# UoB-HPC/pbf-sph

Measured on AMD Instinct MI355X. Metric: particle-steps/sec (1 M particles, 4 iters) + achieved HBM GB/s, 1/2/4/8 MI355X, higher is better.
Workload: dtype f32; 1 GPU; dam-break, 1024000 particles (nominal 1048576), box 4600^3, h=0.1, K=4, dt=0.01245, scale=500; timed = simulation frames [200, 2687) after 195 settle + 5 warm-up frames; particles=1024000, solver_iter=4, settle_frames=195, math=precise (IEEE div/sqrt, no contraction), parallelism=1 GPU, device-resident

## Files before the change

include/pbf_hip.h:

```cpp
#ifndef PBF_HIP_H
#define PBF_HIP_H

#include <stddef.h>
#include <stdint.h>

#ifdef __cplusplus
extern "C" {
#endif

#define PBF_ABI_VERSION 1

typedef struct pbf_ctx pbf_ctx;

typedef enum pbf_status {
  PBF_OK = 0,
  PBF_ERR_INVALID = -1,
  PBF_ERR_HIP = -2,
  PBF_ERR_NO_DEVICE = -3,
  PBF_ERR_STATE = -4,
  PBF_ERR_COMM = -5,
} pbf_status;

enum { PBF_TYPE_FLUID = 0, PBF_TYPE_OBSTACLE = 1 };

// ... 50 lines not shown

int pbf_stage_predict(pbf_ctx *ctx, const pbf_params *params);
int pbf_stage_sort(pbf_ctx *ctx, const pbf_params *params);
int pbf_stage_diffuse(pbf_ctx *ctx, const pbf_params *params);
int pbf_stage_lambda(pbf_ctx *ctx, const pbf_params *params);
int pbf_stage_delta(pbf_ctx *ctx, const pbf_params *params);
int pbf_stage_finalise(pbf_ctx *ctx, const pbf_params *params);

enum pbf_buffer {
  PBF_BUF_KEYS = 0,
  PBF_BUF_TABLE = 1,
  PBF_BUF_PSTAR = 2,
  PBF_BUF_NBR_COUNT = 3,
  PBF_BUF_OMEGA = 4,
  PBF_BUF_SURFACE = 5,
  PBF_BUF_COUNT_ = 6,
};
int pbf_read_buffer(pbf_ctx *ctx, int which, void *host, size_t bytes);
size_t pbf_table_size(const pbf_ctx *ctx);
int pbf_grid_extent(const pbf_ctx *ctx, uint64_t extent[3], double min_extent[3]);

int pbf_selftest_math(pbf_ctx *ctx, uint64_t mismatches[4]);

int pbf_stage_times(pbf_ctx *ctx, const char **names, double *mean_ms, uint64_t *calls, int cap);
int pbf_reset_stage_times(pbf_ctx *ctx);

typedef struct pbf_mc_params {
  double resolution, isolevel, particle_size, particle_influence;
} pbf_mc_params;
int pbf_surface(pbf_ctx *ctx, const pbf_params *params, const pbf_mc_params *mc, uint64_t *n_triangles);
int pbf_download_mesh(pbf_ctx *ctx, void *vs, void *ns, void *cs);
// ... 55 lines not shown
```

pbf-sph_amd/capi.py:

```python
import ctypes as C
import os
import subprocess

import numpy as np

PKG_DIR = os.path.dirname(os.path.abspath(__file__))
LIB_PATH = os.environ.get("PBF_HIP_LIB") or os.path.join(PKG_DIR, "libpbf_hip.so")

ABI_VERSION = 1
FLAG_STAGE_TIMING = 1 << 0
FLAG_FAST_MATH = 1 << 1
FLAG_NO_LDS = 1 << 2

BUF_KEYS, BUF_TABLE, BUF_PSTAR = 0, 1, 2
BUF_NBR_COUNT = 3
BUF_OMEGA = 4
BUF_SURFACE = 5


class PbfError(RuntimeError):
    pass


class Desc(C.Structure):
    _fields_ = [
        ("abi_version", C.c_uint32),
        ("fp64", C.c_int32),
        ("device", C.c_int32),
        ("flags", C.c_uint32),
        ("h", C.c_double),
        ("stream", C.c_void_p),
    ]
# ... 278 lines not shown
    def nbr_counts(self):
        k = np.empty(self.n, np.uint32)
        self._chk(self.L.pbf_read_buffer(self.ctx, BUF_NBR_COUNT, _vp(k), k.nbytes), "read neighbour counts")
        return np.where(k == 0xFFFFFFFF, k, k & 0xFF).astype(np.uint32)

    def keys(self):
        k = np.empty(self.n, np.uint32)
        self._chk(self.L.pbf_read_buffer(self.ctx, BUF_KEYS, _vp(k), k.nbytes), "read keys")
        return k

    def table(self):
        t = np.empty(self.L.pbf_table_size(self.ctx), np.uint32)
        self._chk(self.L.pbf_read_buffer(self.ctx, BUF_TABLE, _vp(t), t.nbytes), "read table")
        return t

    def pstar(self):
        a = np.empty((self.n, 4), self.dtype)
        self._chk(self.L.pbf_read_buffer(self.ctx, BUF_PSTAR, _vp(a), a.nbytes), "read pstar")
        return a

    def omega(self):
        a = np.empty((self.n, 4), self.dtype)
        self._chk(self.L.pbf_read_buffer(self.ctx, BUF_OMEGA, _vp(a), a.nbytes), "read omega")
        return a[:, :3].copy()

    def surface(self, p, mc=None):
        mc = mc or McParams()
        nt = C.c_uint64()
        self._chk(self.L.pbf_surface(self.ctx, C.byref(p), C.byref(mc), C.byref(nt)), "pbf_surface")
        n = nt.value
# ... 25 lines not shown
```

pbf-sph_amd/csrc/pbf_hip.hip:

```cpp
#include "pbf_hip.h"

#include <hip/hip_runtime.h>

#include <cmath>
#include <cstdio>
#include <cstdlib>
#include <cstring>
#include <algorithm>
#include <map>
#include <string>
#include <vector>

#include "pbf_kernels.hpp"
#include "pbf_slab.hpp"
#include "pbf_tiles.hpp"
#include "pbf_mc.hpp"
#include "pbf_comm.hpp"

using namespace pbf;

namespace {

thread_local std::string g_create_error;

struct DevBuf {
  void *p = nullptr;
  size_t cap = 0;
  template <typename T> T *as() const { return static_cast<T *>(p); }
};

constexpr uint32_t kTickets = 254;
constexpr int kBrickZ = 4;

enum Stage { ST_PREDICT = 0, ST_SORT, ST_DIFFUSE, ST_LAMBDA, ST_DELTA, ST_FINALISE, ST_BUILD, ST_COUNT };
const char *kStageNames[ST_COUNT] = {"advect+zindex",      "sortz+gridtable", "sph-diffuse",
                                     "sph-lambda",         "sph-delta",       "sph-finalise",
                                     "sph-lambda/list-build"};

struct EventPair {
  hipEvent_t a, b;
  int stage;
};

}

struct StepState {
// ... 274 lines not shown

int ensure_table(pbf_ctx *ctx, uint32_t tableN) {
  const size_t entries = size_t(tableN) + 2;
  if (ctx->tableCap >= entries) return PBF_OK;
  ctx->count.cap = 0;
  if (ctx->count.p) {
    HIPCHK(ctx, hipStreamSynchronize(ctx->stream));
    HIPCHK(ctx, hipFree(ctx->count.p));
    ctx->count.p = nullptr;
  }
  if (int rc = ensure(ctx, ctx->count, (entries + SCAN_TILE) * 4, true)) return rc;
  if (int rc = ensure(ctx, ctx->table, (entries + SCAN_TILE) * 4)) return rc;
  const size_t nb = (entries + SCAN_TILE - 1) / SCAN_TILE + 1;
  if (int rc = ensure(ctx, ctx->blockSums, nb * 4)) return rc;
  if (int rc = ensure(ctx, ctx->bricks, (entries / Brick<kBrickZ>::HOME + 2) * 4)) return rc;
  if (int rc = ensure(ctx, ctx->brickCtl, (kTickets + 2) * 4)) return rc;
  ctx->tableCap = ctx->count.cap / 4 - SCAN_TILE;
  return PBF_OK;
}

hipEvent_t get_event(pbf_ctx *ctx) {
  if (!ctx->freeEvents.empty()) {
    hipEvent_t e = ctx->freeEvents.back();
    ctx->freeEvents.pop_back();
    return e;
  }
  hipEvent_t e = nullptr;
  (void)hipEventCreate(&e);
  return e;
}
int resolve_events(pbf_ctx *ctx) {
// ... 92 lines not shown
  ctx->bricksValid = true;
}

void launch_scans(pbf_ctx *ctx, const ScanJobs &jobs, int njobs, uint32_t *zero = nullptr, uint32_t nZero = 0) {
  const uint32_t blocks = jobs.nb[0] + (njobs > 1 ? jobs.nb[1] : 0u);
  hipLaunchKernelGGL(k_scan_block_sums, dim3(blocks), dim3(BLOCK), 0, ctx->stream, jobs);
  hipLaunchKernelGGL(k_scan_sums, dim3(uint32_t(njobs)), dim3(BLOCK), 0, ctx->stream, jobs, zero, nZero);
  hipLaunchKernelGGL(k_scan_apply, dim3(blocks), dim3(BLOCK), 0, ctx->stream, jobs);
}
ScanJobs scan_job(const uint32_t *count, uint32_t len, uint32_t *sums, uint32_t *table) {
  ScanJobs j{};
  j.count[0] = count, j.sums[0] = sums, j.table[0] = table, j.len[0] = len, j.nb[0] = (len + SCAN_TILE - 1) / SCAN_TILE;
  return j;
}

template <typename N> int stage_sort(pbf_ctx *ctx, const pbf_params *p) {
  if (!ctx->counted) return fail(ctx, PBF_ERR_STATE, "pbf_stage_sort needs pbf_stage_predict first");
  StepConsts<N> c;
  if (int rc = make_consts<N>(ctx, p, c)) return rc;
  if (c.tableN != ctx->countedTableN) return fail(ctx, PBF_ERR_STATE, "bounds changed between predict and sort");
  StageTimer t(ctx, ST_SORT);
  const uint32_t len = c.tableN + 2;
  const uint32_t nb = (len + SCAN_TILE - 1) / SCAN_TILE;
  uint32_t *count = ctx->count.as<uint32_t>(), *table = ctx->table.as<uint32_t>(),
           *sums = ctx->blockSums.as<uint32_t>();
  ScanJobs jobs = scan_job(count, len, sums, table);
  int njobs = 1;
  (void)nb;
  const int s = ctx->cur, d = 1 - s;
  RowArrays<N> row{};
  ctx->rowsValid = false, ctx->pstarInRows = false, ctx->rowsCurrent = false, ctx->rowColValid = false;
  if (row_mode(ctx)) {
    uint32_t pshift = 1;
    while (pshift < 10 && (uint64_t(1) << (3 * pshift)) < uint64_t(c.tableN)) ++pshift;
    const size_t ncells = size_t(1) << (3 * pshift), llen = ncells + 1;
    const uint32_t lnb = uint32_t((llen + SCAN_TILE - 1) / SCAN_TILE);
    const size_t v = sizeof(vec4<N>);
    if (int rc = ensure(ctx, ctx->linCount, (ncells + 2 + SCAN_TILE) * 4)) return rc;
    if (int rc = ensure(ctx, ctx->linTable, (ncells + 2 + SCAN_TILE) * 4)) return rc;
    if (int rc = ensure(ctx, ctx->linSums, (size_t(lnb) + 2) * 4)) return rc;
    for (int k = 0; k < 2; ++k)
      if (int rc = ensure(ctx, ctx->rowPstar[k], ctx->cap * v)) return rc;
    if (int rc = ensure(ctx, ctx->rowMass, ctx->cap * sizeof(N))) return rc;
    if (int rc = ensure(ctx, ctx->rowQpos, (ctx->cap + QPOS_PAD) * 8)) return rc;
    if (int rc = ensure(ctx, ctx->rowXYZ, ctx->cap * 4)) return rc;
    if (int rc = ensure(ctx, ctx->rowType, ctx->cap)) return rc;
    if (int rc = ensure(ctx, ctx->rowSlotOf, ctx->cap * 4)) return rc;
    const bool rowDiffuse = ctx->cellDiffuse && ctx->rowDiffuse > 0;
    const uint32_t segShift = std::min<uint32_t>(pshift, 6u);
    const size_t nSegTotal = ncells >> segShift;
    if (rowDiffuse) {
      if (int rc = ensure(ctx, ctx->rowCol, ctx->cap * v)) return rc;
      if (int rc = ensure(ctx, ctx->rowMortonOf, ctx->cap * 4)) return rc;
      if (int rc = ensure(ctx, ctx->rowSegs, (std::min(nSegTotal, ctx->cap) + 1) * 4)) return rc;
    }
    hipLaunchKernelGGL(k_lin_count, grid_for(ncells + 1), dim3(BLOCK), 0, ctx->stream, c.tableN, pshift, count,
                       ctx->linCount.as<uint32_t>());
    jobs.count[1] = ctx->linCount.as<const uint32_t>(), jobs.sums[1] = ctx->linSums.as<uint32_t>(), jobs.table[1] = ctx->linTable.as<uint32_t>();
    jobs.len[1] = uint32_t(llen), jobs.nb[1] = lnb;
    njobs = 2;
    launch_scans(ctx, jobs, njobs, ctx->brickCtl.as<uint32_t>(), kTickets + 2);
    if (rowDiffuse)
      hipLaunchKernelGGL(k_row_segments, grid_for(nSegTotal), dim3(BLOCK), 0, ctx->stream, pshift, segShift,
                         ctx->linTable.as<const uint32_t>(), ctx->rowSegs.as<uint32_t>(), ctx->linCount.as<uint32_t>() + ncells + 2);
    ctx->rcur = 0;
    row = RowArrays<N>{ctx->rowPstar[0].as<vec4<N>>(), ctx->rowMass.as<N>(), ctx->rowQpos.as<uint2>(), ctx->rowXYZ.as<uint32_t>(),
                       ctx->rowType.as<uint8_t>(), ctx->rowSlotOf.as<uint32_t>(),
                       rowDiffuse ? ctx->rowCol.as<vec4<N>>() : nullptr, rowDiffuse ? ctx->rowMortonOf.as<uint32_t>() : nullptr,
                       ctx->linTable.as<const uint32_t>(), ctx->linCount.as<uint32_t>() + ncells + 1, pshift};
    ctx->rowShift = pshift, ctx->rowSegShift = segShift;
    ctx->rowColValid = rowDiffuse;
    ctx->rowsValid = true, ctx->rowsCurrent = true;
  }
  if (njobs == 1) launch_scans(ctx, jobs, 1, ctx->brickCtl.as<uint32_t>(), kTickets + 2);
  uint32_t *nBig = ctx->brickCtl.as<uint32_t>() + kTickets + 1;
  if (int rc = ensure(ctx, ctx->bigCells, (ctx->cap / BIG_CELL + 2) * 4)) return rc;
  hipLaunchKernelGGL(k_scatter_slots, grid_for(ctx->n), dim3(BLOCK), 0, ctx->stream, c.n, c.tableN,
                     ctx->key[s].as<const uint32_t>(), table, count, ctx->permTmp.as<uint32_t>(),
                     ctx->bigCells.as<uint32_t>(), nBig);
  hipLaunchKernelGGL(k_sort_big_cells, dim3(64), dim3(BLOCK), 0, ctx->stream, table, c.tableN,
                     ctx->bigCells.as<const uint32_t>(), nBig, ctx->permTmp.as<uint32_t>(),
                     ctx->key[s].as<const uint32_t>());
  const size_t nLive = ctx->slabStepMode ? ctx->sortLive : ctx->n;
  hipLaunchKernelGGL((k_rank_move<N>), grid_for(nLive), dim3(BLOCK), 0, ctx->stream, c, uint32_t(nLive), c.tableN,
                     ctx->permTmp.as<const uint32_t>(), table, arrays<N>(ctx, s, s), arrays<N>(ctx, d, d),
                     ctx->slabActive ? ctx->slotOf.as<uint32_t>() : nullptr, ctx->qpos.as<uint2>(), row);
  ctx->n = nLive;
  ctx->gatherSeq = 0;
  ctx->bricksValid = false;
  if (!ctx->rowColValid) brick_list(ctx, c.tableN, true);
  LAUNCH_CHECK(ctx);
  ctx->cur = d;
  ctx->pcur = d;
  ctx->sorted = true;
  ctx->nbrValid = false;
  ctx->qposValid = true;
  if (ctx->rowsValid) ctx->pstarInRows = true, ctx->qposValid = false;
  ctx->counted = false;
  return PBF_OK;
}
// ... 158 lines not shown
  return PBF_OK;
}

template <typename N> int stage_diffuse(pbf_ctx *ctx, const pbf_params *p, bool overlap = false) {
  StepConsts<N> c;
  if (int rc = make_consts<N>(ctx, p, c)) return rc;
  const int s = ctx->cur, d = 1 - s;
  typename DiffuseOp<N>::Args args{ctx->col4[s].as<const vec4<N>>(), ctx->col4[d].as<vec4<N>>(),
                                   ctx->type[s].as<const uint8_t>()};
  const bool timed = (ctx->desc.flags & PBF_FLAG_STAGE_TIMING) != 0 && ((ctx->timingMask >> ST_DIFFUSE) & 1u) != 0;
  overlap = overlap && ctx->overlapDiffuse && ctx->cellDiffuse && !(ctx->desc.flags & PBF_FLAG_NO_LDS) && !timed &&
            (ctx->overlapDiffuseForced || ctx->n >= (size_t(1) << 19));
  ctx->omegaValid = false, ctx->surfaceValid = false;
  StageTimer t(ctx, ST_DIFFUSE);
  if (ctx->cellDiffuse && ctx->rowColValid && ctx->rowsValid && ctx->rowDiffuse) {
    const uint32_t ncells = 1u << (3u * ctx->rowShift);
    const uint32_t cap = ctx->diffuseCap ? ctx->diffuseCap : 640u;
    const size_t lds = size_t(cap + 8) * sizeof(vec4<N>) + size_t(DIFFUSE_ROW_THREADS) * (4 * sizeof(N) + 4) + cap + 8;
    static size_t attrSet = 0;
    if (lds > attrSet) {
      (void)hipFuncSetAttribute(reinterpret_cast<const void *>(k_diffuse_rows<N>), hipFuncAttributeMaxDynamicSharedMemorySize, int(lds));
      attrSet = lds;
    }
    const uint32_t perCU = uint32_t(std::max<size_t>(1, std::min<size_t>(16, (160 * 1024) / (lds + 256))));
    const uint32_t blocks = std::max(8u, (uint32_t(ctx->numCUs) * perCU) & ~7u);
    hipLaunchKernelGGL((k_diffuse_rows<N>), dim3(blocks), dim3(DIFFUSE_ROW_THREADS), lds, ctx->stream, c,
                       row_walk<N>(ctx), ctx->rowCol.as<const vec4<N>>(), ctx->rowType.as<const uint8_t>(),
                       ctx->rowMortonOf.as<const uint32_t>(), ctx->rowSegs.as<const uint32_t>(),
                       ctx->linCount.as<const uint32_t>() + ncells + 2, ctx->rowSegShift, args.colOut, cap, uint32_t(ctx->n));
    LAUNCH_CHECK(ctx);
    ctx->rowColValid = false;
  } else if (ctx->cellDiffuse && !(ctx->desc.flags & PBF_FLAG_NO_LDS)) {
    brick_list(ctx, c.tableN);
    vec4<N> *cellSum = ctx->pstar[other_pstar(ctx)].as<vec4<N>>();
    uint32_t *cellCnt = ctx->nbrCount.as<uint32_t>();
    hipStream_t st = ctx->stream;
    uint32_t cap = 3072u;
    if (overlap) cap = 2048u;
    const size_t lds = Brick<4>::HDR + size_t(cap) * sizeof(vec4<N>);
    uint32_t perCU = uint32_t((160 * 1024) / (lds + 1024));
    if (overlap) {
      if (int rc = ensure(ctx, ctx->diffSum, ctx->cap * sizeof(vec4<N>))) return rc;
      if (int rc = ensure(ctx, ctx->diffCnt, ctx->cap * 4)) return rc;
      if (!ctx->sideStream) {
// ... 243 lines not shown
    std::swap(ctx->pstar[ctx->pcur], ctx->pstar[s]);
    ctx->pcur = s;
  }
  ctx->nbrValid = false;
  if (extras_on(ctx, p)) return extras<N>(ctx, p, c);
  return PBF_OK;
}

template <typename N> int step_impl(pbf_ctx *ctx, const pbf_params *p) {
  if (ctx->n == 0) return PBF_OK;
  if (ctx->prePredicted) {
    ctx->prePredicted = false;
  } else if (int rc = stage_predict<N>(ctx, p)) {
    return rc;
  }
  if (int rc = stage_sort<N>(ctx, p)) return rc;
  const bool fuse = ctx->fuseDiffuse && p->iteration > 0 && ctx->gatherKind == 1 && ctx->reuseLists &&
                    !(ctx->desc.flags & PBF_FLAG_NO_LDS);
  if (!fuse) {
    if (int rc = stage_diffuse<N>(ctx, p, p->iteration > 0)) return rc;
  }
  ctx->fuseDiffuseNow = fuse;
  for (uint64_t it = 0; it < p->iteration; ++it) {
    if (int rc = stage_lambda<N>(ctx, p)) return rc;
    if (int rc = stage_delta<N>(ctx, p)) return rc;
  }
  if (int rc = stage_finalise<N>(ctx, p)) return rc;
  return join_diffuse(ctx);
}

int check(pbf_ctx *ctx, const pbf_params *p, bool needSorted) {
  if (!ctx) return PBF_ERR_INVALID;
  if (!p) return fail(ctx, PBF_ERR_INVALID, "params == NULL");
// ... 542 lines not shown
      src = ctx->table.p, avail = size_t(ctx->tableN) * 4;
      break;
    case PBF_BUF_PSTAR:
      if (int rc = ctx->fp64 ? materialise_pstar<double>(ctx) : materialise_pstar<float>(ctx)) return rc;
      src = ctx->pstar[ctx->pcur].p, avail = ctx->n * v;
      break;
    case PBF_BUF_NBR_COUNT: src = ctx->nbrCount.p, avail = (ctx->ghostsPending ? ctx->nOwned : ctx->n) * 4; break;
    case PBF_BUF_OMEGA:
      if (!ctx->omegaValid) return fail(ctx, PBF_ERR_STATE, "no vorticity pass since the arrays last changed (pbf_params.vorticity)");
      src = ctx->pstar[2].p, avail = ctx->n * v;
      break;
    case PBF_BUF_SURFACE:
      if (!ctx->surfaceValid) return fail(ctx, PBF_ERR_STATE, "no surface-tension pass since the arrays last changed (pbf_set_surface_tension)");
      src = ctx->surfB.p, avail = std::min(ctx->n * v, ctx->surfB.cap);
      break;
    default: return fail(ctx, PBF_ERR_INVALID, "unknown buffer");
  }
  if (bytes > avail) return fail(ctx, PBF_ERR_INVALID, "read beyond buffer");
  if (!src) return fail(ctx, PBF_ERR_STATE, "buffer not allocated yet");
  HIPCHK(ctx, hipMemcpyAsync(host, src, bytes, hipMemcpyDeviceToHost, ctx->stream));
  HIPCHK(ctx, hipStreamSynchronize(ctx->stream));
  return PBF_OK;
}

int pbf_selftest_math(pbf_ctx *ctx, uint64_t mismatches[4]) {
  if (!ctx || !mismatches) return PBF_ERR_INVALID;
  HIPCHK(ctx, hipSetDevice(ctx->device));
  if (int rc = ensure(ctx, ctx->selTotals, 64)) return rc;
  HIPCHK(ctx, hipMemsetAsync(ctx->selTotals.p, 0, 32, ctx->stream));
  if (ctx->fp64) {
// ... 808 lines not shown
```

pbf-sph_amd/csrc/pbf_kernels.hpp:

```cpp
#pragma once

#include <type_traits>

#include "pbf_common.hpp"

namespace pbf {

constexpr int BLOCK = 256;

template <typename N> __device__ inline int64_t cell_coord(N v) {
  return static_cast<int64_t>(v);
}

template <typename F> __device__ inline void wave_bucket_atomic(uint32_t bucket, F &&leader_op, uint32_t &before, uint32_t &rank) {
  const uint32_t lane = threadIdx.x & 63u;
  const uint64_t below = (1ull << lane) - 1ull;
  bool pending = true;
  uint32_t cnt = 0, leader = lane;
  rank = 0;
  while (__any(pending)) {
    if (pending) {
      const uint32_t b = __builtin_amdgcn_readfirstlane(bucket);
      if (bucket == b) {
        const uint64_t same = __ballot(1);
// ... 107 lines not shown
  const uint32_t incl = wave_incl_scan(v, lane);
  __syncthreads();
  if (lane == 63) waveSum[wave] = incl;
  __syncthreads();
  uint32_t off = 0, tot = 0;
#pragma unroll
  for (int w = 0; w < THREADS / 64; ++w) {
    const uint32_t s = waveSum[w];
    if (w < wave) off += s;
    tot += s;
  }
  *total = tot;
  return off + incl - v;
}

struct ScanJobs {
  const uint32_t *count[2];
  uint32_t *sums[2];
  uint32_t *table[2];
  uint32_t len[2], nb[2];
};
__global__ __launch_bounds__(BLOCK) void k_scan_block_sums(ScanJobs jobs) {
  const uint32_t j = blockIdx.x >= jobs.nb[0] ? 1u : 0u, blk = blockIdx.x - (j ? jobs.nb[0] : 0u);
  const uint32_t *__restrict__ count = jobs.count[j];
  const uint32_t len = jobs.len[j];
  const uint32_t base = blk * SCAN_TILE + threadIdx.x * SCAN_ITEMS;
  uint32_t s = 0;
  if (base + SCAN_ITEMS <= len) {
    const uint4 a = *reinterpret_cast<const uint4 *>(count + base);
    const uint4 b = *reinterpret_cast<const uint4 *>(count + base + 4);
    s = a.x + a.y + a.z + a.w + b.x + b.y + b.z + b.w;
  } else {
    for (int k = 0; k < SCAN_ITEMS; ++k)
      if (base + k < len) s += count[base + k];
  }
  uint32_t total;
  block_excl_scan(s, &total);
  if (threadIdx.x == 0) jobs.sums[j][blk] = total;
}

__global__ __launch_bounds__(BLOCK) void k_scan_sums(ScanJobs jobs, uint32_t *__restrict__ zero, uint32_t nZero) {
  if (blockIdx.x == 0)
    for (uint32_t k = threadIdx.x; k < nZero; k += BLOCK) zero[k] = 0u;
  uint32_t *__restrict__ blockSums = jobs.sums[blockIdx.x];
  const uint32_t nb = jobs.nb[blockIdx.x];
  uint32_t carry = 0;
  for (uint32_t base = 0; base < nb; base += BLOCK) {
    const uint32_t i = base + threadIdx.x;
    const uint32_t v = i < nb ? blockSums[i] : 0u;
    uint32_t total;
    const uint32_t ex = block_excl_scan(v, &total);
    if (i < nb) blockSums[i] = carry + ex;
    carry += total;
  }
}

__global__ __launch_bounds__(BLOCK) void k_scan_apply(ScanJobs jobs) {
  const uint32_t j = blockIdx.x >= jobs.nb[0] ? 1u : 0u, blk = blockIdx.x - (j ? jobs.nb[0] : 0u);
  const uint32_t *__restrict__ count = jobs.count[j];
  uint32_t *__restrict__ table = jobs.table[j];
  const uint32_t len = jobs.len[j];
  const uint32_t base = blk * SCAN_TILE + threadIdx.x * SCAN_ITEMS;
  uint32_t v[SCAN_ITEMS];
  uint32_t s = 0;
#pragma unroll
  for (int k = 0; k < SCAN_ITEMS; ++k) {
    v[k] = (base + k < len) ? count[base + k] : 0u;
    s += v[k];
  }
  uint32_t total;
  uint32_t run = block_excl_scan(s, &total) + jobs.sums[j][blk];
#pragma unroll
  for (int k = 0; k < SCAN_ITEMS; ++k) {
    if (base + k < len) table[base + k] = run;
    run += v[k];
  }
}

constexpr int QPOS_BITS = 11;
constexpr uint32_t QPOS_T = (1u << QPOS_BITS) + 5;
typedef short qpair __attribute__((ext_vector_type(2)));

template <typename N> __device__ inline uint2 quantise_position(const StepConsts<N> &c, const vec4<N> &p, bool *usable) {
  const N k = N(1u << QPOS_BITS) / c.h;
  const N fx = floor((p.x - c.minExtent[0]) * k), fy = floor((p.y - c.minExtent[1]) * k),
          fz = floor((p.z - c.minExtent[2]) * k);
  const N lim = N(1 << 22);
  *usable = fabs(fx) < lim && fabs(fy) < lim && fabs(fz) < lim;
  const uint32_t x = uint32_t(int32_t(fx)), y = uint32_t(int32_t(fy)), z = uint32_t(int32_t(fz));
  return make_uint2((x & 0xFFFFu) | (y << 16), z & 0xFFFFu);
}


constexpr uint32_t BIG_CELL = 2048;

__global__ __launch_bounds__(BLOCK) void k_scatter_slots(uint32_t n, uint32_t tableN, const uint32_t *__restrict__ key,
                                                         const uint32_t *__restrict__ table,
                                                         uint32_t *__restrict__ count,
                                                         uint32_t *__restrict__ permTmp,
                                                         uint32_t *__restrict__ bigCells,
                                                         uint32_t *__restrict__ nBig) {
  const uint32_t i = blockIdx.x * BLOCK + threadIdx.x;
  if (i >= n) return;
  const uint32_t k = key[i];
  if (k == DEAD_KEY) return;
  const uint32_t b = min(k, tableN);
  uint32_t before, rank;
  wave_bucket_atomic(b, [&](uint32_t bb, uint32_t cnt) { return atomicSub(&count[bb], cnt); }, before, rank);
  const uint32_t r = before - 1u - rank;
  permTmp[table[b] + r] = i;
  if (r == BIG_CELL) bigCells[atomicAdd(nBig, 1u)] = b;
}

__global__ __launch_bounds__(BLOCK) void k_sort_big_cells(const uint32_t *__restrict__ table, uint32_t tableN,
                                                          const uint32_t *__restrict__ bigCells,
                                                          const uint32_t *__restrict__ nBig,
                                                          uint32_t *__restrict__ permTmp,
                                                          const uint32_t *__restrict__ key) {
  const uint32_t cells = *nBig;
  for (uint32_t c = blockIdx.x; c < cells; c += gridDim.x) {
    const uint32_t b = bigCells[c];
    const uint32_t lo = table[b], m = table[b + 1] - lo;
    uint32_t *a = permTmp + lo;
    const bool byKey = b == tableN;
    auto exchange = [&](uint32_t i, uint32_t l) {
      const uint32_t x = a[i], y = a[l];
      bool swap;
      if (byKey) {
        const uint32_t kx = key[x], ky = key[y];
        swap = ky < kx || (ky == kx && y < x);
      } else {
        swap = y < x;
      }
      if (swap) a[i] = y, a[l] = x;
    };
// ... 2 lines not shown
    for (uint32_t k = 2; k <= P; k <<= 1) {
      for (uint32_t i = threadIdx.x; i < m; i += BLOCK) {
        const uint32_t l = i ^ (k - 1u);
        if (l > i && l < m) exchange(i, l);
      }
      __syncthreads();
      for (uint32_t j = k >> 2; j > 0; j >>= 1) {
        for (uint32_t i = threadIdx.x; i < m; i += BLOCK) {
          const uint32_t l = i ^ j;
          if (l > i && l < m) exchange(i, l);
        }
        __syncthreads();
      }
    }
  }
}

template <typename N> struct ParticleArrays {
  vec4<N> *pos4, *vel4, *col4, *pstar;
  uint64_t *id;
  uint8_t *type;
  uint32_t *key;
};

constexpr uint32_t ROW_FALLBACK = 1u << 30;
template <typename N> struct RowArrays {
  vec4<N> *pstar;
  N *mass;
  uint2 *qpos;
  uint32_t *xyz;
  uint8_t *type;
  uint32_t *slotOf;
  vec4<N> *col;
  uint32_t *mortonOf;
  const uint32_t *lintab;
  uint32_t *tail;
  uint32_t pshift;
};
__host__ __device__ inline bool row_cell_of(uint32_t key, uint32_t tableN, uint32_t pshift, uint32_t *lin) {
  const uint32_t x = compact10(key), y = compact10(key >> 1), z = compact10(key >> 2);
  *lin = (((z << pshift) | y) << pshift) | x;
  return key + 1u < tableN;
}

__global__ __launch_bounds__(BLOCK) void k_lin_count(uint32_t tableN, uint32_t pshift, const uint32_t *__restrict__ count,
                                                     uint32_t *__restrict__ linCount) {
  const uint32_t code = blockIdx.x * BLOCK + threadIdx.x;
  if (code >= (1u << (3u * pshift))) {
    if (code == (1u << (3u * pshift))) linCount[code] = 0u, linCount[code + 1u] = 0u, linCount[code + 2u] = 0u;
    return;
  }
  uint32_t lin;
  const bool known = row_cell_of(code, tableN, pshift, &lin);
  linCount[lin] = known ? count[code] : 0u;
}

template <typename N>
__global__ __launch_bounds__(BLOCK) void k_rank_move(StepConsts<N> c, uint32_t n, uint32_t tableN,
                                                     const uint32_t *__restrict__ permTmp,
                                                     const uint32_t *__restrict__ table, ParticleArrays<N> src,
                                                     ParticleArrays<N> dst, uint32_t *__restrict__ slotOf,
                                                     uint2 *__restrict__ qpos, RowArrays<N> row) {
  const uint32_t i = blockIdx.x * BLOCK + threadIdx.x;
  if (i >= n) return;
  const uint32_t s = permTmp[i];
  const uint32_t k = src.key[s];
  const uint32_t b = min(k, tableN);
  const uint32_t lo = table[b], hi = table[b + 1];
  uint32_t rank = 0;
  if (hi - lo > BIG_CELL) {
    rank = i - lo;
  } else if (b < tableN) {
    for (uint32_t j = lo; j < hi; j += 4u) {
      uint32_t v[4];
#pragma unroll
      for (uint32_t k = 0; k < 4; ++k) v[k] = permTmp[min(j + k, hi - 1u)];
#pragma unroll
      for (uint32_t k = 0; k < 4; ++k) rank += (j + k < hi && v[k] < s) ? 1u : 0u;
    }
  } else {
    for (uint32_t j = lo; j < hi; ++j) {
      const uint32_t sj = permTmp[j];
      const uint32_t kj = src.key[sj];
      rank += (kj < k || (kj == k && sj < s)) ? 1u : 0u;
    }
  }
  const uint32_t d = lo + rank;
  const vec4<N> p4 = src.pos4[s];
  dst.pos4[d] = p4;
  dst.vel4[d] = src.vel4[s];
  const vec4<N> cl = src.col4[s];
  dst.col4[d] = cl;
  const vec4<N> ps = src.pstar[s];
  bool usable;
  const uint2 q = quantise_position<N>(c, ps, &usable);
  if (!row.lintab) {
    dst.pstar[d] = ps;
    qpos[d] = q;
  }
  dst.id[d] = src.id[s];
  const uint8_t ty = src.type[s];
  dst.type[d] = ty;
  dst.key[d] = k;
  if (slotOf) slotOf[s] = d;
  if (row.lintab) {
    uint32_t lin, slot;
    const uint32_t x = compact10(k), y = compact10(k >> 1), z = compact10(k >> 2);
    uint32_t flags = 0;
    if (row_cell_of(k, tableN, row.pshift, &lin)) {
      slot = row.lintab[lin] + rank;
      if (row.pshift == 10u && (x == 0u || y == 0u || z == 0u || x == 1023u || y == 1023u || z == 1023u)) flags = ROW_FALLBACK;
    } else {
      slot = row.lintab[1u << (3u * row.pshift)] + atomicAdd(row.tail, 1u);
      flags = ROW_FALLBACK;
    }
    row.pstar[slot] = ps, row.mass[slot] = p4.w, row.qpos[slot] = q, row.type[slot] = ty;
    row.xyz[slot] = x | (y << 10) | (z << 20) | flags;
    row.slotOf[d] = slot;
    if (row.col) row.col[slot] = cl, row.mortonOf[slot] = d;
  }
}

struct Neigh {
  uint32_t xs[3], ys[3], zs[3];
};
// ... 1177 lines not shown
    for_each_candidate(morton_encode(x, y, z), w.mtable, w.tableN, [&](uint32_t b) { f(w.slotOf[b]); });
    return;
  }
#pragma unroll 1
  for (uint32_t r = 0; r < 9; ++r) {
    const RowRun run = row_run(w, x, y, z, r);
    for (uint32_t b = run.s; b < run.e; ++b) f(b);
  }
}

constexpr int DIFFUSE_ROW_THREADS = 64;
__device__ inline void lds_dma16(const void *src, void *ldsBase) {
  using G = const __attribute__((address_space(1))) void *;
  using L = __attribute__((address_space(3))) void *;
  __builtin_amdgcn_global_load_lds((G)(uintptr_t)src, (L)(uint32_t)(uintptr_t)ldsBase, 16, 0, 0);
}
__global__ __launch_bounds__(BLOCK) void k_row_segments(uint32_t pshift, uint32_t segShift, const uint32_t *__restrict__ lintab,
                                                        uint32_t *__restrict__ segs, uint32_t *__restrict__ nSegs) {
  const uint32_t sg = blockIdx.x * BLOCK + threadIdx.x;
  if (sg >= (1u << (3u * pshift - segShift))) return;
  const uint32_t c0 = sg << segShift;
  if (lintab[c0 + (1u << segShift)] != lintab[c0]) segs[atomicAdd(nSegs, 1u)] = sg;
}

template <typename N>
__global__ __launch_bounds__(DIFFUSE_ROW_THREADS) void k_diffuse_rows(StepConsts<N> c, RowWalk rw, const vec4<N> *__restrict__ rowCol,
                                                                      const uint8_t *__restrict__ rowType,
                                                                      const uint32_t *__restrict__ mortonOf,
                                                                      const uint32_t *__restrict__ segs,
                                                                      const uint32_t *__restrict__ nSegsPtr, uint32_t segShift,
                                                                      vec4<N> *__restrict__ colOut, uint32_t cap, uint32_t nSlots) {
  constexpr uint32_t T = DIFFUSE_ROW_THREADS;
  constexpr uint32_t UNITS = sizeof(vec4<N>) / 16u;
  extern __shared__ __align__(16) unsigned char smem[];
  vec4<N> *tile = reinterpret_cast<vec4<N> *>(smem);
  N *sums = reinterpret_cast<N *>(smem + size_t(cap + 8u) * sizeof(vec4<N>));
  uint32_t *cnts = reinterpret_cast<uint32_t *>(sums + 4 * T);
// ... 614 lines not shown
```

Measured before the change: 866.2 million particle-steps/s.

## Fold row-count, segment and big-cell passes into scan and scatter kernels

```diff
diff --git a/include/pbf_hip.h b/include/pbf_hip.h
--- a/include/pbf_hip.h
+++ b/include/pbf_hip.h
@@ -88,7 +88,11 @@
   PBF_BUF_NBR_COUNT = 3,
   PBF_BUF_OMEGA = 4,
   PBF_BUF_SURFACE = 5,
-  PBF_BUF_COUNT_ = 6,
+  PBF_BUF_ROW_TABLE = 6,
+  PBF_BUF_ROW_SEGS = 7,
+  PBF_BUF_ROW_SLOT_OF = 8,
+  PBF_BUF_ROW_MORTON_OF = 9,
+  PBF_BUF_COUNT_ = 10,
 };
 int pbf_read_buffer(pbf_ctx *ctx, int which, void *host, size_t bytes);
 size_t pbf_table_size(const pbf_ctx *ctx);
diff --git a/pbf-sph_amd/capi.py b/pbf-sph_amd/capi.py
--- a/pbf-sph_amd/capi.py
+++ b/pbf-sph_amd/capi.py
@@ -16,6 +16,7 @@
 BUF_NBR_COUNT = 3
 BUF_OMEGA = 4
 BUF_SURFACE = 5
+BUF_ROW_TABLE, BUF_ROW_SEGS, BUF_ROW_SLOT_OF, BUF_ROW_MORTON_OF = 6, 7, 8, 9
 
 
 class PbfError(RuntimeError):
@@ -324,6 +325,28 @@
         self._chk(self.L.pbf_read_buffer(self.ctx, BUF_TABLE, _vp(t), t.nbytes), "read table")
         return t
 
+    def row_tables(self):
+        ts = self.L.pbf_table_size(self.ctx)
+        ps = 1
+        while ps < 10 and 8 ** ps < ts:
+            ps += 1
+        out = {"pshift": ps}
+        t = np.empty(8 ** ps + 1, np.uint32)
+        self._chk(self.L.pbf_read_buffer(self.ctx, BUF_ROW_TABLE, _vp(t), t.nbytes), "read row table")
+        out["table"] = t
+        a = np.empty(self.n, np.uint32)
+        self._chk(self.L.pbf_read_buffer(self.ctx, BUF_ROW_SLOT_OF, _vp(a), a.nbytes), "read row slots")
+        out["slot_of"] = a
+        m = np.empty(1, np.uint32)
+        if self.L.pbf_read_buffer(self.ctx, BUF_ROW_SEGS, _vp(m), 4) == 0:
+            g = np.empty(1 + int(m[0]), np.uint32)
+            self._chk(self.L.pbf_read_buffer(self.ctx, BUF_ROW_SEGS, _vp(g), g.nbytes), "read row segments")
+            out["segs"] = np.sort(g[1:])
+            b = np.empty(self.n, np.uint32)
+            self._chk(self.L.pbf_read_buffer(self.ctx, BUF_ROW_MORTON_OF, _vp(b), b.nbytes), "read row Morton indices")
+            out["morton_of"] = b
+        return out
+
     def pstar(self):
         a = np.empty((self.n, 4), self.dtype)
         self._chk(self.L.pbf_read_buffer(self.ctx, BUF_PSTAR, _vp(a), a.nbytes), "read pstar")
diff --git a/pbf-sph_amd/csrc/pbf_hip.hip b/pbf-sph_amd/csrc/pbf_hip.hip
--- a/pbf-sph_amd/csrc/pbf_hip.hip
+++ b/pbf-sph_amd/csrc/pbf_hip.hip
@@ -30,6 +30,8 @@
 };
 
 constexpr uint32_t kTickets = 254;
+constexpr uint32_t kCtlBigCells = kTickets + 1, kCtlBigTotal = kTickets + 2, kCtlBigArrived = kTickets + 3,
+                   kCtlRowTail = kTickets + 4, kCtlRowSegs = kTickets + 5, kCtlWords = kTickets + 6;
 constexpr int kBrickZ = 4;
 
 enum Stage { ST_PREDICT = 0, ST_SORT, ST_DIFFUSE, ST_LAMBDA, ST_DELTA, ST_FINALISE, ST_BUILD, ST_COUNT };
@@ -334,7 +336,7 @@
   const size_t nb = (entries + SCAN_TILE - 1) / SCAN_TILE + 1;
   if (int rc = ensure(ctx, ctx->blockSums, nb * 4)) return rc;
   if (int rc = ensure(ctx, ctx->bricks, (entries / Brick<kBrickZ>::HOME + 2) * 4)) return rc;
-  if (int rc = ensure(ctx, ctx->brickCtl, (kTickets + 2) * 4)) return rc;
+  if (int rc = ensure(ctx, ctx->brickCtl, kCtlWords * 4)) return rc;
   ctx->tableCap = ctx->count.cap / 4 - SCAN_TILE;
   return PBF_OK;
 }
@@ -457,19 +459,19 @@
   return j;
 }
 
-template <typename N> int stage_sort(pbf_ctx *ctx, const pbf_params *p) {
+template <typename N> int stage_sort(pbf_ctx *ctx, const pbf_params *p, bool diffuseNext = false) {
   if (!ctx->counted) return fail(ctx, PBF_ERR_STATE, "pbf_stage_sort needs pbf_stage_predict first");
   StepConsts<N> c;
   if (int rc = make_consts<N>(ctx, p, c)) return rc;
   if (c.tableN != ctx->countedTableN) return fail(ctx, PBF_ERR_STATE, "bounds changed between predict and sort");
   StageTimer t(ctx, ST_SORT);
   const uint32_t len = c.tableN + 2;
-  const uint32_t nb = (len + SCAN_TILE - 1) / SCAN_TILE;
   uint32_t *count = ctx->count.as<uint32_t>(), *table = ctx->table.as<uint32_t>(),
-           *sums = ctx->blockSums.as<uint32_t>();
+           *sums = ctx->blockSums.as<uint32_t>(), *ctl = ctx->brickCtl.as<uint32_t>();
   ScanJobs jobs = scan_job(count, len, sums, table);
+  if (int rc = ensure(ctx, ctx->bigCells, (ctx->cap / BIG_CELL + 2) * 4)) return rc;
+  jobs.bigCells = ctx->bigCells.as<uint32_t>(), jobs.nBig = ctl + kCtlBigCells, jobs.bigTotal = ctl + kCtlBigTotal;
   int njobs = 1;
-  (void)nb;
   const int s = ctx->cur, d = 1 - s;
   RowArrays<N> row{};
   ctx->rowsValid = false, ctx->pstarInRows = false, ctx->rowsCurrent = false, ctx->rowColValid = false;
@@ -496,37 +498,30 @@
       if (int rc = ensure(ctx, ctx->rowCol, ctx->cap * v)) return rc;
       if (int rc = ensure(ctx, ctx->rowMortonOf, ctx->cap * 4)) return rc;
       if (int rc = ensure(ctx, ctx->rowSegs, (std::min(nSegTotal, ctx->cap) + 1) * 4)) return rc;
+      jobs.segs = ctx->rowSegs.as<uint32_t>(), jobs.nSegs = ctl + kCtlRowSegs, jobs.segShift = segShift;
     }
-    hipLaunchKernelGGL(k_lin_count, grid_for(ncells + 1), dim3(BLOCK), 0, ctx->stream, c.tableN, pshift, count,
-                       ctx->linCount.as<uint32_t>());
+    jobs.hist = count, jobs.rowCount = ctx->linCount.as<uint32_t>();
     jobs.count[1] = ctx->linCount.as<const uint32_t>(), jobs.sums[1] = ctx->linSums.as<uint32_t>(), jobs.table[1] = ctx->linTable.as<uint32_t>();
-    jobs.len[1] = uint32_t(llen), jobs.nb[1] = lnb;
+    jobs.len[1] = uint32_t(llen), jobs.nb[1] = lnb, jobs.rowShift = pshift, jobs.tableN = c.tableN;
     njobs = 2;
-    launch_scans(ctx, jobs, njobs, ctx->brickCtl.as<uint32_t>(), kTickets + 2);
-    if (rowDiffuse)
-      hipLaunchKernelGGL(k_row_segments, grid_for(nSegTotal), dim3(BLOCK), 0, ctx->stream, pshift, segShift,
-                         ctx->linTable.as<const uint32_t>(), ctx->rowSegs.as<uint32_t>(), ctx->linCount.as<uint32_t>() + ncells + 2);
     ctx->rcur = 0;
     row = RowArrays<N>{ctx->rowPstar[0].as<vec4<N>>(), ctx->rowMass.as<N>(), ctx->rowQpos.as<uint2>(), ctx->rowXYZ.as<uint32_t>(),
                        ctx->rowType.as<uint8_t>(), ctx->rowSlotOf.as<uint32_t>(),
                        rowDiffuse ? ctx->rowCol.as<vec4<N>>() : nullptr, rowDiffuse ? ctx->rowMortonOf.as<uint32_t>() : nullptr,
-                       ctx->linTable.as<const uint32_t>(), ctx->linCount.as<uint32_t>() + ncells + 1, pshift};
+                       ctx->linTable.as<const uint32_t>(), ctl + kCtlRowTail, pshift};
     ctx->rowShift = pshift, ctx->rowSegShift = segShift;
     ctx->rowColValid = rowDiffuse;
     ctx->rowsValid = true, ctx->rowsCurrent = true;
   }
-  if (njobs == 1) launch_scans(ctx, jobs, 1, ctx->brickCtl.as<uint32_t>(), kTickets + 2);
-  uint32_t *nBig = ctx->brickCtl.as<uint32_t>() + kTickets + 1;
-  if (int rc = ensure(ctx, ctx->bigCells, (ctx->cap / BIG_CELL + 2) * 4)) return rc;
+  launch_scans(ctx, jobs, njobs, ctl, kCtlWords);
   hipLaunchKernelGGL(k_scatter_slots, grid_for(ctx->n), dim3(BLOCK), 0, ctx->stream, c.n, c.tableN,
                      ctx->key[s].as<const uint32_t>(), table, count, ctx->permTmp.as<uint32_t>(),
-                     ctx->bigCells.as<uint32_t>(), nBig);
-  hipLaunchKernelGGL(k_sort_big_cells, dim3(64), dim3(BLOCK), 0, ctx->stream, table, c.tableN,
-                     ctx->bigCells.as<const uint32_t>(), nBig, ctx->permTmp.as<uint32_t>(),
-                     ctx->key[s].as<const uint32_t>());
+                     ctx->bigCells.as<const uint32_t>(), ctl + kCtlBigCells, ctl + kCtlBigTotal, ctl + kCtlBigArrived);
   const size_t nLive = ctx->slabStepMode ? ctx->sortLive : ctx->n;
+  ParticleArrays<N> dstArr = arrays<N>(ctx, d, d);
+  if (diffuseNext && ctx->rowColValid && !ctx->slabActive && !ctx->slabStepMode) dstArr.col4 = nullptr;
   hipLaunchKernelGGL((k_rank_move<N>), grid_for(nLive), dim3(BLOCK), 0, ctx->stream, c, uint32_t(nLive), c.tableN,
-                     ctx->permTmp.as<const uint32_t>(), table, arrays<N>(ctx, s, s), arrays<N>(ctx, d, d),
+                     ctx->permTmp.as<const uint32_t>(), table, arrays<N>(ctx, s, s), dstArr,
                      ctx->slabActive ? ctx->slotOf.as<uint32_t>() : nullptr, ctx->qpos.as<uint2>(), row);
   ctx->n = nLive;
   ctx->gatherSeq = 0;
@@ -715,7 +710,6 @@
   ctx->omegaValid = false, ctx->surfaceValid = false;
   StageTimer t(ctx, ST_DIFFUSE);
   if (ctx->cellDiffuse && ctx->rowColValid && ctx->rowsValid && ctx->rowDiffuse) {
-    const uint32_t ncells = 1u << (3u * ctx->rowShift);
     const uint32_t cap = ctx->diffuseCap ? ctx->diffuseCap : 640u;
     const size_t lds = size_t(cap + 8) * sizeof(vec4<N>) + size_t(DIFFUSE_ROW_THREADS) * (4 * sizeof(N) + 4) + cap + 8;
     static size_t attrSet = 0;
@@ -728,7 +722,7 @@
     hipLaunchKernelGGL((k_diffuse_rows<N>), dim3(blocks), dim3(DIFFUSE_ROW_THREADS), lds, ctx->stream, c,
                        row_walk<N>(ctx), ctx->rowCol.as<const vec4<N>>(), ctx->rowType.as<const uint8_t>(),
                        ctx->rowMortonOf.as<const uint32_t>(), ctx->rowSegs.as<const uint32_t>(),
-                       ctx->linCount.as<const uint32_t>() + ncells + 2, ctx->rowSegShift, args.colOut, cap, uint32_t(ctx->n));
+                       ctx->brickCtl.as<const uint32_t>() + kCtlRowSegs, ctx->rowSegShift, args.colOut, cap, uint32_t(ctx->n));
     LAUNCH_CHECK(ctx);
     ctx->rowColValid = false;
   } else if (ctx->cellDiffuse && !(ctx->desc.flags & PBF_FLAG_NO_LDS)) {
@@ -1002,9 +996,9 @@
   } else if (int rc = stage_predict<N>(ctx, p)) {
     return rc;
   }
-  if (int rc = stage_sort<N>(ctx, p)) return rc;
   const bool fuse = ctx->fuseDiffuse && p->iteration > 0 && ctx->gatherKind == 1 && ctx->reuseLists &&
                     !(ctx->desc.flags & PBF_FLAG_NO_LDS);
+  if (int rc = stage_sort<N>(ctx, p, !fuse)) return rc;
   if (!fuse) {
     if (int rc = stage_diffuse<N>(ctx, p, p->iteration > 0)) return rc;
   }
@@ -1577,6 +1571,30 @@
       if (!ctx->surfaceValid) return fail(ctx, PBF_ERR_STATE, "no surface-tension pass since the arrays last changed (pbf_set_surface_tension)");
       src = ctx->surfB.p, avail = std::min(ctx->n * v, ctx->surfB.cap);
       break;
+    case PBF_BUF_ROW_TABLE:
+    case PBF_BUF_ROW_SEGS:
+    case PBF_BUF_ROW_SLOT_OF:
+    case PBF_BUF_ROW_MORTON_OF: {
+      if (!ctx->rowsValid) return fail(ctx, PBF_ERR_STATE, "no row tables for the current sorted set (option row_major)");
+      const bool rowDiffuse = ctx->cellDiffuse && ctx->rowDiffuse > 0;
+      if ((which == PBF_BUF_ROW_SEGS || which == PBF_BUF_ROW_MORTON_OF) && !rowDiffuse)
+        return fail(ctx, PBF_ERR_STATE, "row diffusion is off (options cell_diffuse, row_diffuse)");
+      if (which == PBF_BUF_ROW_TABLE) src = ctx->linTable.p, avail = ((size_t(1) << (3 * ctx->rowShift)) + 1) * 4;
+      if (which == PBF_BUF_ROW_SLOT_OF) src = ctx->rowSlotOf.p, avail = ctx->n * 4;
+      if (which == PBF_BUF_ROW_MORTON_OF) src = ctx->rowMortonOf.p, avail = ctx->n * 4;
+      if (which == PBF_BUF_ROW_SEGS) {
+        uint32_t m = 0;
+        HIPCHK(ctx, hipMemcpyAsync(&m, ctx->brickCtl.as<uint32_t>() + kCtlRowSegs, 4, hipMemcpyDeviceToHost, ctx->stream));
+        HIPCHK(ctx, hipStreamSynchronize(ctx->stream));
+        if (bytes < 4) return fail(ctx, PBF_ERR_INVALID, "read beyond buffer");
+        if (bytes > (size_t(m) + 1) * 4) return fail(ctx, PBF_ERR_INVALID, "read beyond buffer");
+        std::memcpy(host, &m, 4);
+        host = static_cast<char *>(host) + 4, bytes -= 4;
+        src = ctx->rowSegs.p, avail = size_t(m) * 4;
+        if (bytes == 0) return PBF_OK;
+      }
+      break;
+    }
     default: return fail(ctx, PBF_ERR_INVALID, "unknown buffer");
   }
   if (bytes > avail) return fail(ctx, PBF_ERR_INVALID, "read beyond buffer");
diff --git a/pbf-sph_amd/csrc/pbf_kernels.hpp b/pbf-sph_amd/csrc/pbf_kernels.hpp
--- a/pbf-sph_amd/csrc/pbf_kernels.hpp
+++ b/pbf-sph_amd/csrc/pbf_kernels.hpp
@@ -145,26 +145,77 @@
   return off + incl - v;
 }
 
+constexpr uint32_t BIG_CELL = 2048;
 struct ScanJobs {
   const uint32_t *count[2];
   uint32_t *sums[2];
   uint32_t *table[2];
   uint32_t len[2], nb[2];
-};
-__global__ __launch_bounds__(BLOCK) void k_scan_block_sums(ScanJobs jobs) {
-  const uint32_t j = blockIdx.x >= jobs.nb[0] ? 1u : 0u, blk = blockIdx.x - (j ? jobs.nb[0] : 0u);
+  const uint32_t *hist;
+  uint32_t *rowCount;
+  uint32_t rowShift, tableN, segShift;
+  uint32_t *segs, *nSegs;
+  uint32_t *bigCells, *nBig, *bigTotal;
+};
+__device__ inline void scan_load(const ScanJobs &jobs, uint32_t j, uint32_t base, uint32_t (&v)[SCAN_ITEMS]) {
   const uint32_t *__restrict__ count = jobs.count[j];
   const uint32_t len = jobs.len[j];
-  const uint32_t base = blk * SCAN_TILE + threadIdx.x * SCAN_ITEMS;
-  uint32_t s = 0;
   if (base + SCAN_ITEMS <= len) {
     const uint4 a = *reinterpret_cast<const uint4 *>(count + base);
     const uint4 b = *reinterpret_cast<const uint4 *>(count + base + 4);
-    s = a.x + a.y + a.z + a.w + b.x + b.y + b.z + b.w;
+    v[0] = a.x, v[1] = a.y, v[2] = a.z, v[3] = a.w, v[4] = b.x, v[5] = b.y, v[6] = b.z, v[7] = b.w;
   } else {
-    for (int k = 0; k < SCAN_ITEMS; ++k)
-      if (base + k < len) s += count[base + k];
-  }
+#pragma unroll
+    for (int k = 0; k < SCAN_ITEMS; ++k) v[k] = (base + uint32_t(k) < len) ? count[base + k] : 0u;
+  }
+}
+__device__ inline void row_gather(const ScanJobs &jobs, uint32_t base, uint32_t (&v)[SCAN_ITEMS]) {
+  const uint32_t *__restrict__ hist = jobs.hist;
+  const uint32_t ps = jobs.rowShift, m = (1u << ps) - 1u, ncells = 1u << (3u * ps);
+  const uint32_t c0 = morton_encode(base & m, (base >> ps) & m, base >> (2u * ps));
+  if (ps >= 3u && base < ncells && c0 + 74u < jobs.tableN) {
+    constexpr uint32_t off[4] = {0u, 8u, 64u, 72u};
+#pragma unroll
+    for (int q = 0; q < 4; ++q) {
+      const uint2 w = *reinterpret_cast<const uint2 *>(hist + c0 + off[q]);
+      v[2 * q] = w.x, v[2 * q + 1] = w.y;
+    }
+    return;
+  }
+#pragma unroll
+  for (int k = 0; k < SCAN_ITEMS; ++k) {
+    const uint32_t lin = base + uint32_t(k);
+    v[k] = 0u;
+    if (lin < ncells) {
+      const uint32_t code = morton_encode(lin & m, (lin >> ps) & m, lin >> (2u * ps));
+      if (code + 1u < jobs.tableN) v[k] = hist[code];
+    }
+  }
+}
+static_assert(SCAN_ITEMS == 8, "scan_load / k_scan_apply move a thread's items as two 16-byte vectors");
+
+__global__ __launch_bounds__(BLOCK) void k_scan_block_sums(ScanJobs jobs) {
+  const uint32_t j = blockIdx.x >= jobs.nb[0] ? 1u : 0u, blk = blockIdx.x - (j ? jobs.nb[0] : 0u);
+  const uint32_t base = blk * SCAN_TILE + threadIdx.x * SCAN_ITEMS;
+  uint32_t v[SCAN_ITEMS];
+  if (j == 1u && jobs.rowShift != 0u) {
+    row_gather(jobs, base, v);
+    const uint32_t len = jobs.len[1];
+    uint32_t *__restrict__ rc = jobs.rowCount;
+    if (base + SCAN_ITEMS <= len) {
+      *reinterpret_cast<uint4 *>(rc + base) = make_uint4(v[0], v[1], v[2], v[3]);
+      *reinterpret_cast<uint4 *>(rc + base + 4) = make_uint4(v[4], v[5], v[6], v[7]);
+    } else {
+#pragma unroll
+      for (int k = 0; k < SCAN_ITEMS; ++k)
+        if (base + uint32_t(k) < len) rc[base + k] = v[k];
+    }
+  } else {
+    scan_load(jobs, j, base, v);
+  }
+  uint32_t s = 0;
+#pragma unroll
+  for (int k = 0; k < SCAN_ITEMS; ++k) s += v[k];
   uint32_t total;
   block_excl_scan(s, &total);
   if (threadIdx.x == 0) jobs.sums[j][blk] = total;
@@ -188,23 +239,60 @@
 
 __global__ __launch_bounds__(BLOCK) void k_scan_apply(ScanJobs jobs) {
   const uint32_t j = blockIdx.x >= jobs.nb[0] ? 1u : 0u, blk = blockIdx.x - (j ? jobs.nb[0] : 0u);
-  const uint32_t *__restrict__ count = jobs.count[j];
   uint32_t *__restrict__ table = jobs.table[j];
   const uint32_t len = jobs.len[j];
   const uint32_t base = blk * SCAN_TILE + threadIdx.x * SCAN_ITEMS;
   uint32_t v[SCAN_ITEMS];
+  scan_load(jobs, j, base, v);
   uint32_t s = 0;
 #pragma unroll
-  for (int k = 0; k < SCAN_ITEMS; ++k) {
-    v[k] = (base + k < len) ? count[base + k] : 0u;
-    s += v[k];
-  }
+  for (int k = 0; k < SCAN_ITEMS; ++k) s += v[k];
   uint32_t total;
   uint32_t run = block_excl_scan(s, &total) + jobs.sums[j][blk];
-#pragma unroll
-  for (int k = 0; k < SCAN_ITEMS; ++k) {
-    if (base + k < len) table[base + k] = run;
-    run += v[k];
+  uint32_t t[SCAN_ITEMS];
+#pragma unroll
+  for (int k = 0; k < SCAN_ITEMS; ++k) t[k] = run, run += v[k];
+  if (base + SCAN_ITEMS <= len) {
+    *reinterpret_cast<uint4 *>(table + base) = make_uint4(t[0], t[1], t[2], t[3]);
+    *reinterpret_cast<uint4 *>(table + base + 4) = make_uint4(t[4], t[5], t[6], t[7]);
+  } else {
+#pragma unroll
+    for (int k = 0; k < SCAN_ITEMS; ++k)
+      if (base + uint32_t(k) < len) table[base + k] = t[k];
+  }
+  if (j == 0u && jobs.bigCells) {
+#pragma unroll
+    for (int k = 0; k < SCAN_ITEMS; ++k)
+      if (v[k] > BIG_CELL) jobs.bigCells[atomicAdd(jobs.nBig, 1u)] = base + k, atomicAdd(jobs.bigTotal, v[k]);
+  }
+  if (j == 1u && jobs.segs) {
+    const uint32_t sh = jobs.segShift, lane = threadIdx.x & 63u, wave = threadIdx.x >> 6;
+    if (sh >= 3u) {
+      const uint32_t G = 1u << (sh - 3u);
+      const uint64_t occ = __ballot(s != 0u);
+      const bool lead = (lane & (G - 1u)) == 0u && ((occ >> lane) & ((1ull << G) - 1ull)) != 0ull;
+      const uint64_t leads = __ballot(lead);
+      __shared__ uint32_t waveAt[BLOCK / 64], blockAt;
+      if (lane == 0u) waveAt[wave] = uint32_t(__builtin_popcountll(leads));
+      __syncthreads();
+      if (threadIdx.x == 0) {
+        uint32_t tot = 0;
+        for (int w = 0; w < BLOCK / 64; ++w) {
+          const uint32_t c = waveAt[w];
+          waveAt[w] = tot, tot += c;
+        }
+        blockAt = tot ? atomicAdd(jobs.nSegs, tot) : 0u;
+      }
+      __syncthreads();
+      if (lead) jobs.segs[blockAt + waveAt[wave] + uint32_t(__builtin_popcountll(leads & ((1ull << lane) - 1ull)))] = base >> sh;
+    } else {
+      const uint32_t X = 1u << sh;
+      for (uint32_t k = 0; k < SCAN_ITEMS; k += X) {
+        uint32_t m = 0;
+        for (uint32_t q = 0; q < X; ++q) m += v[k + q];
+        if (m != 0u) jobs.segs[atomicAdd(jobs.nSegs, 1u)] = (base + k) >> sh;
+      }
+    }
   }
 }
 
@@ -223,33 +311,10 @@
 }
 
 
-constexpr uint32_t BIG_CELL = 2048;
-
-__global__ __launch_bounds__(BLOCK) void k_scatter_slots(uint32_t n, uint32_t tableN, const uint32_t *__restrict__ key,
-                                                         const uint32_t *__restrict__ table,
-                                                         uint32_t *__restrict__ count,
-                                                         uint32_t *__restrict__ permTmp,
-                                                         uint32_t *__restrict__ bigCells,
-                                                         uint32_t *__restrict__ nBig) {
-  const uint32_t i = blockIdx.x * BLOCK + threadIdx.x;
-  if (i >= n) return;
-  const uint32_t k = key[i];
-  if (k == DEAD_KEY) return;
-  const uint32_t b = min(k, tableN);
-  uint32_t before, rank;
-  wave_bucket_atomic(b, [&](uint32_t bb, uint32_t cnt) { return atomicSub(&count[bb], cnt); }, before, rank);
-  const uint32_t r = before - 1u - rank;
-  permTmp[table[b] + r] = i;
-  if (r == BIG_CELL) bigCells[atomicAdd(nBig, 1u)] = b;
-}
-
-__global__ __launch_bounds__(BLOCK) void k_sort_big_cells(const uint32_t *__restrict__ table, uint32_t tableN,
-                                                          const uint32_t *__restrict__ bigCells,
-                                                          const uint32_t *__restrict__ nBig,
-                                                          uint32_t *__restrict__ permTmp,
-                                                          const uint32_t *__restrict__ key) {
-  const uint32_t cells = *nBig;
-  for (uint32_t c = blockIdx.x; c < cells; c += gridDim.x) {
+
+__device__ inline void sort_big_cells(const uint32_t *__restrict__ table, uint32_t tableN, const uint32_t *__restrict__ bigCells,
+                                      uint32_t cells, uint32_t *__restrict__ permTmp, const uint32_t *__restrict__ key) {
+  for (uint32_t c = 0; c < cells; ++c) {
     const uint32_t b = bigCells[c];
     const uint32_t lo = table[b], m = table[b + 1] - lo;
     uint32_t *a = permTmp + lo;
@@ -282,6 +347,38 @@
       }
     }
   }
+}
+
+__global__ __launch_bounds__(BLOCK) void k_scatter_slots(uint32_t n, uint32_t tableN, const uint32_t *__restrict__ key,
+                                                         const uint32_t *__restrict__ table,
+                                                         uint32_t *__restrict__ count,
+                                                         uint32_t *__restrict__ permTmp,
+                                                         const uint32_t *__restrict__ bigCells,
+                                                         const uint32_t *__restrict__ nBig,
+                                                         const uint32_t *__restrict__ bigTotal,
+                                                         uint32_t *__restrict__ bigArrived) {
+  const uint32_t i = blockIdx.x * BLOCK + threadIdx.x;
+  const uint32_t k = i < n ? key[i] : DEAD_KEY;
+  bool big = false;
+  if (k != DEAD_KEY) {
+    const uint32_t b = min(k, tableN);
+    uint32_t before, rank;
+    wave_bucket_atomic(b, [&](uint32_t bb, uint32_t cnt) { return atomicSub(&count[bb], cnt); }, before, rank);
+    const uint32_t r = before - 1u - rank;
+    const uint32_t lo = table[b];
+    permTmp[lo + r] = i;
+    big = table[b + 1] - lo > BIG_CELL;
+  }
+  const uint32_t nb = __syncthreads_count(big);
+  if (nb == 0u) return;
+  __threadfence();
+  __syncthreads();
+  __shared__ uint32_t last;
+  if (threadIdx.x == 0) last = atomicAdd(bigArrived, nb) + nb == *bigTotal ? 1u : 0u;
+  __syncthreads();
+  if (!last) return;
+  __threadfence();
+  sort_big_cells(table, tableN, bigCells, *nBig, permTmp, key);
 }
 
 template <typename N> struct ParticleArrays {
@@ -311,28 +408,22 @@
   return key + 1u < tableN;
 }
 
-__global__ __launch_bounds__(BLOCK) void k_lin_count(uint32_t tableN, uint32_t pshift, const uint32_t *__restrict__ count,
-                                                     uint32_t *__restrict__ linCount) {
-  const uint32_t code = blockIdx.x * BLOCK + threadIdx.x;
-  if (code >= (1u << (3u * pshift))) {
-    if (code == (1u << (3u * pshift))) linCount[code] = 0u, linCount[code + 1u] = 0u, linCount[code + 2u] = 0u;
-    return;
-  }
-  uint32_t lin;
-  const bool known = row_cell_of(code, tableN, pshift, &lin);
-  linCount[lin] = known ? count[code] : 0u;
-}
-
 template <typename N>
 __global__ __launch_bounds__(BLOCK) void k_rank_move(StepConsts<N> c, uint32_t n, uint32_t tableN,
                                                      const uint32_t *__restrict__ permTmp,
                                                      const uint32_t *__restrict__ table, ParticleArrays<N> src,
                                                      ParticleArrays<N> dst, uint32_t *__restrict__ slotOf,
                                                      uint2 *__restrict__ qpos, RowArrays<N> row) {
-  const uint32_t i = blockIdx.x * BLOCK + threadIdx.x;
+  const uint32_t i = xcd_chunk() * BLOCK + threadIdx.x;
   if (i >= n) return;
   const uint32_t s = permTmp[i];
   const uint32_t k = src.key[s];
+  const vec4<N> p4 = src.pos4[s], v4 = src.vel4[s], cl = src.col4[s], ps = src.pstar[s];
+  const uint64_t id = src.id[s];
+  const uint8_t ty = src.type[s];
+  uint32_t lin = 0, rowBase = 0;
+  const bool inCell = row.lintab && row_cell_of(k, tableN, row.pshift, &lin);
+  if (inCell) rowBase = row.lintab[lin];
   const uint32_t b = min(k, tableN);
   const uint32_t lo = table[b], hi = table[b + 1];
   uint32_t rank = 0;
@@ -354,29 +445,25 @@
     }
   }
   const uint32_t d = lo + rank;
-  const vec4<N> p4 = src.pos4[s];
   dst.pos4[d] = p4;
-  dst.vel4[d] = src.vel4[s];
-  const vec4<N> cl = src.col4[s];
-  dst.col4[d] = cl;
-  const vec4<N> ps = src.pstar[s];
+  dst.vel4[d] = v4;
+  if (dst.col4) dst.col4[d] = cl;
   bool usable;
   const uint2 q = quantise_position<N>(c, ps, &usable);
   if (!row.lintab) {
     dst.pstar[d] = ps;
     qpos[d] = q;
   }
-  dst.id[d] = src.id[s];
-  const uint8_t ty = src.type[s];
+  dst.id[d] = id;
   dst.type[d] = ty;
   dst.key[d] = k;
   if (slotOf) slotOf[s] = d;
   if (row.lintab) {
-    uint32_t lin, slot;
+    uint32_t slot;
     const uint32_t x = compact10(k), y = compact10(k >> 1), z = compact10(k >> 2);
     uint32_t flags = 0;
-    if (row_cell_of(k, tableN, row.pshift, &lin)) {
-      slot = row.lintab[lin] + rank;
+    if (inCell) {
+      slot = rowBase + rank;
       if (row.pshift == 10u && (x == 0u || y == 0u || z == 0u || x == 1023u || y == 1023u || z == 1023u)) flags = ROW_FALLBACK;
     } else {
       slot = row.lintab[1u << (3u * row.pshift)] + atomicAdd(row.tail, 1u);
@@ -1584,13 +1671,6 @@
   using G = const __attribute__((address_space(1))) void *;
   using L = __attribute__((address_space(3))) void *;
   __builtin_amdgcn_global_load_lds((G)(uintptr_t)src, (L)(uint32_t)(uintptr_t)ldsBase, 16, 0, 0);
-}
-__global__ __launch_bounds__(BLOCK) void k_row_segments(uint32_t pshift, uint32_t segShift, const uint32_t *__restrict__ lintab,
-                                                        uint32_t *__restrict__ segs, uint32_t *__restrict__ nSegs) {
-  const uint32_t sg = blockIdx.x * BLOCK + threadIdx.x;
-  if (sg >= (1u << (3u * pshift - segShift))) return;
-  const uint32_t c0 = sg << segShift;
-  if (lintab[c0 + (1u << segShift)] != lintab[c0]) segs[atomicAdd(nSegs, 1u)] = sg;
 }
 
 template <typename N>
```

New measurement: 890.3 million particle-steps/s (median of 6 runs). 1.03x the previous value.
